# lijun9250lj/video-steganography-PCAMV

Measured on AMD Instinct MI355X. Metric: 1080p macroblocks/s (embed on), higher is better.
Workload: dtype u8

## Files before the change

### include/pcamv_gpu.h

```cpp
#ifndef PCAMV_GPU_H
#define PCAMV_GPU_H

#include <stddef.h>
#include <stdint.h>

#ifdef __cplusplus
extern "C" {
#endif

#define PCAMV_EINVAL  (-1)
#define PCAMV_ENODEV  (-2)
#define PCAMV_ENOMEM  (-3)
#define PCAMV_EHIP    (-4)
#define PCAMV_EUNSUP  (-5)

enum { PCAMV_ME_DIA = 0, PCAMV_ME_HEX = 1, PCAMV_ME_UMH = 2, PCAMV_ME_ESA = 3, PCAMV_ME_TESA = 4 };
enum { PCAMV_P_L0 = 4, PCAMV_P_8x8 = 5, PCAMV_P_SKIP = 6 };
enum { PCAMV_D_L0_4x4 = 0, PCAMV_D_L0_8x4 = 1, PCAMV_D_L0_4x8 = 2, PCAMV_D_L0_8x8 = 3,
       PCAMV_D_8x8 = 13, PCAMV_D_16x8 = 14, PCAMV_D_8x16 = 15, PCAMV_D_16x16 = 16 };
#define PCAMV_ANALYSE_I4x4      0x0001u
#define PCAMV_ANALYSE_PSUB16x16 0x0010u
#define PCAMV_ANALYSE_PSUB8x8   0x0020u

typedef struct pcamv_params_t {
    int32_t i_width, i_height;
    int32_t i_me_method;
    int32_t i_me_range;
    int32_t i_subpel_refine;
    int32_t i_mv_range;
    int32_t b_chroma_me;
    int32_t b_fast_pskip;
    int32_t b_dct_decimate;
    int32_t b_cabac;
    uint32_t inter;
    int32_t i_chroma_qp_offset;
    int32_t i_luma_deadzone[2];
    int32_t i_tscale;
    int32_t i_psy_rd;
} pcamv_params_t;

typedef struct pcamv_mb_t {
    int32_t i_type;
    int32_t i_partition;
    int32_t i_qp;
    uint8_t i_sub_partition[4];
    int8_t  ref[16];
    int16_t mv[16][2];
    int16_t mv_stego[16][2];
    int32_t inter_stego_cost[16];
    int16_t pskip_mv[2];
    int16_t mvr16[2];
    uint8_t used;
    uint8_t pad[3];
} pcamv_mb_t;

typedef struct pcamv_embed_t {
    int32_t  n;
    int32_t  m;
    int32_t  stc_ok;
    int32_t  num_flip;
    uint8_t *cover;
    float   *rho;
    uint8_t *message;
    uint8_t *stego;
    int8_t  *flip;
} pcamv_embed_t;

typedef struct pcamv_ctx pcamv_ctx_t;
typedef struct pcamv_batch pcamv_batch_t;

int  pcamv_gpu_open(const pcamv_params_t *param, int device, pcamv_ctx_t **ctx);
void pcamv_gpu_close(pcamv_ctx_t *ctx);
const char *pcamv_gpu_last_error(const pcamv_ctx_t *ctx);

int pcamv_gpu_upload_fenc(pcamv_ctx_t *ctx, const uint8_t *const plane[3], const int stride[3]);

int pcamv_gpu_set_ref(pcamv_ctx_t *ctx, const uint8_t *const plane[3], const int stride[3],
                      const int16_t *prev_mv, const int8_t *prev_ref);

int pcamv_gpu_get_ref_planes(pcamv_ctx_t *ctx, uint8_t *out, int *stride, int *lines);

int pcamv_gpu_analyse_pframe(pcamv_ctx_t *ctx, int qp, int embed, pcamv_mb_t *out_mb,
                             uint8_t *const recon[3]);

int pcamv_gpu_embed_pframe(pcamv_ctx_t *ctx, float emrate, const uint8_t *message, int message_len,
                           pcamv_embed_t *out);

int pcamv_gpu_final_mvs(pcamv_ctx_t *ctx, pcamv_mb_t *out_mb);

int pcamv_gpu_pass2_pframe(pcamv_ctx_t *ctx, const uint8_t *flips, int n_flips, pcamv_mb_t *out_final,
                           uint8_t *const recon[3], uint8_t *const deblocked[3]);

int pcamv_gpu_stc_extract(const uint8_t *stego, int n, int m, int matrixheight, uint8_t *message);
int pcamv_gpu_stc_extract_lcg(const uint8_t *stego, int n, int m, int matrixheight, int64_t *lcg, uint8_t *message);

int pcamv_gpu_parse_pslice_cabac(const uint8_t *slice_data, size_t len, int mb_w, int mb_h, int slice_qp, pcamv_mb_t *out_mb);
int pcamv_gpu_parse_pslice_cavlc(const uint8_t *slice_data, size_t len, int mb_w, int mb_h, pcamv_mb_t *out_mb);
int pcamv_gpu_nal_to_rbsp(const uint8_t *nal, size_t len, uint8_t *rbsp, size_t *rbsp_len, int *nal_ref_idc, int *nal_unit_type);
int pcamv_gpu_parse_pslice_cabac_at(const uint8_t *rbsp, size_t len, size_t start_bit, int mb_w, int mb_h, int slice_qp, pcamv_mb_t *out_mb);
int pcamv_gpu_parse_pslice_cavlc_at(const uint8_t *rbsp, size_t len, size_t start_bit, int mb_w, int mb_h, pcamv_mb_t *out_mb);

int pcamv_gpu_set_ref_device(pcamv_ctx_t *ctx, const void *y, const void *u, const void *v,
                             const void *prev_mv, const void *prev_ref);
#define PCAMV_PREV_FIELD_INTERNAL ((const void *)(uintptr_t)1)
int pcamv_gpu_set_fenc_device(pcamv_ctx_t *ctx, const void *y, const void *u, const void *v);
int pcamv_gpu_step_device(pcamv_ctx_t *ctx, int qp, float emrate, void *stream);
int pcamv_gpu_fetch_results(pcamv_ctx_t *ctx, pcamv_mb_t *out_mb, pcamv_embed_t *out);
int  pcamv_gpu_batch_create(pcamv_ctx_t *const *ctxs, int n, pcamv_batch_t **batch);
void pcamv_gpu_batch_destroy(pcamv_batch_t *batch);
int  pcamv_gpu_batch_step(pcamv_batch_t *batch, int qp, float emrate, void *stream);
int  pcamv_gpu_batch_kernel_time(pcamv_batch_t *batch, const char *kernel, double *avg_ms, int *launches, int reset);
const char *pcamv_gpu_batch_last_error(const pcamv_batch_t *batch);
int  pcamv_gpu_batch_set_closed_loop(pcamv_batch_t *batch, int on);
int  pcamv_gpu_recon_device(pcamv_ctx_t *ctx, void *planes[3]);
int  pcamv_gpu_fetch_recon(pcamv_ctx_t *ctx, uint8_t *const planes[3]);
const char *pcamv_gpu_batch_dominant_kernel(const pcamv_batch_t *batch);
int  pcamv_gpu_batch_copy_results_async(pcamv_batch_t *batch, void *dst_mb, size_t mb_stride, void *dst_flip, size_t flip_stride, void *stream);

int pcamv_gpu_kernel_time(pcamv_ctx_t *ctx, const char *kernel, double *avg_ms, int *launches, int reset);

int pcamv_gpu_block_costs(pcamv_ctx_t *ctx, int qp, int n, const int32_t *req, int32_t *out);

int pcamv_gpu_rd_probe(pcamv_ctx_t *ctx, int qp, int n, const uint8_t *req, int32_t *out);

int pcamv_gpu_embed_records(pcamv_ctx_t *ctx, const pcamv_mb_t *mbs, float emrate,
                            const uint8_t *message, int message_len, pcamv_embed_t *out);

int pcamv_gpu_trace_mb(pcamv_ctx_t *ctx, int mb);
int pcamv_gpu_trace_fetch(pcamv_ctx_t *ctx, int32_t *out);

int pcamv_gpu_debug_state_hash(pcamv_ctx_t *ctx, int enable);
int pcamv_gpu_debug_state_hash_fetch(pcamv_ctx_t *ctx, uint32_t *out);

int pcamv_gpu_abi_version(void);
#define PCAMV_FEATURE_PAYLOAD 0x1u
#define PCAMV_FEATURE_SLICE_PARSER 0x2u
#define PCAMV_FEATURE_SLICE_PARSER_CAVLC 0x4u
#define PCAMV_FEATURE_SLICE_WRITER 0x8u
#define PCAMV_FEATURE_SLICE_WRITER_CAVLC 0x10u
unsigned pcamv_gpu_features(void);

int pcamv_gpu_set_payload(pcamv_ctx_t *ctx, const uint8_t *bytes, int64_t n_bits);
int pcamv_gpu_set_payload_device(pcamv_ctx_t *ctx, const void *device_bytes, int64_t n_bits);
int pcamv_gpu_payload_tell(pcamv_ctx_t *ctx, int64_t *consumed_bits, int64_t *payload_bits);

int pcamv_gpu_rx_reserve(pcamv_ctx_t *ctx, int64_t n_bits);
int pcamv_gpu_rx_reset(pcamv_ctx_t *ctx);
int pcamv_gpu_rx_tell(pcamv_ctx_t *ctx, int64_t *received_bits, int64_t *reserved_bits);
int pcamv_gpu_rx_fetch(pcamv_ctx_t *ctx, uint8_t *bytes, int64_t n_bits);
int pcamv_gpu_batch_extract_step(pcamv_batch_t *batch, float emrate, void *stream);
int pcamv_gpu_extract_pframe(pcamv_ctx_t *ctx, const pcamv_mb_t *mbs, float emrate, uint8_t *bits_out, int32_t *n, int32_t *m);
int pcamv_gpu_batch_payload_check(pcamv_batch_t *batch, int64_t *diff);

int pcamv_gpu_parse_pslice_cabac_device(pcamv_ctx_t *ctx, const uint8_t *rbsp, size_t len, size_t start_bit, int slice_qp, pcamv_mb_t *out_mb);
typedef struct pcamv_slice_t { const uint8_t *rbsp; size_t len; size_t start_bit; int32_t slice_qp; } pcamv_slice_t;
int pcamv_gpu_batch_extract_slices(pcamv_batch_t *batch, const pcamv_slice_t *slices, float emrate, void *stream);
int pcamv_gpu_batch_extract_slices_device(pcamv_batch_t *batch, const void *bytes, size_t bytes_size, const int64_t *off, const int64_t *len,
                                          const int64_t *start_bit, const int32_t *slice_qp, float emrate, void *stream);
int pcamv_gpu_batch_slice_status(pcamv_batch_t *batch, int32_t *status);
int pcamv_gpu_debug_slice_records(pcamv_ctx_t *ctx, pcamv_mb_t *out_mb, int *guard_intact);

int pcamv_gpu_parse_pslice_cavlc_device(pcamv_ctx_t *ctx, const uint8_t *rbsp, size_t len, size_t start_bit, pcamv_mb_t *out_mb);
int pcamv_gpu_batch_extract_slices_cavlc(pcamv_batch_t *batch, const pcamv_slice_t *slices, float emrate, void *stream);
// ... 20 lines not shown
```

### video-steganography-pcamv_amd/csrc/pcamv_gpu.hip

```cpp
#include <hip/hip_runtime.h>
#include <math.h>
#include <stdarg.h>
#include <stdio.h>
#include <stdlib.h>
#include <string.h>
#include <new>
#include "pcamv_planes.hip.h"
#include "pcamv_kernels.hip.h"
#include "pcamv_embed.hip.h"
#include "pcamv_slice.hip.h"
#include "pcamv_host_tables.h"
#include "pcamv_mvsyntax.h"
#include "pcamv_rd_select.h"

#define PCAMV_ABI_VERSION 3
#define NEV 32
#define NRING 8
#define NKEV 16
enum { KT_ANALYSE, KT_EMBED_PREPARE, KT_EXTRACT_PREPARE, KT_EXTRACT_BITS, KT_PAYLOAD_CHECK, KT_PARSE_PSLICE, KT_PARSE_PSLICE_CAVLC, KT_WRITE_PSLICE, KT_WRITE_PSLICE_CAVLC, KT_N };
#define PCAMV_FEATURES (PCAMV_FEATURE_PAYLOAD | PCAMV_FEATURE_SLICE_PARSER | PCAMV_FEATURE_SLICE_PARSER_CAVLC | PCAMV_FEATURE_SLICE_WRITER | \
                        PCAMV_FEATURE_SLICE_WRITER_CAVLC)
#define SLICE_GUARD_MBS 4
#define NSTAGE 2
enum { ST_PLANES = 1, ST_ANALYSE = 2, ST_EMBED = 4, ST_PASS2 = 8 };
// ... 518 lines not shown
    *k_out = k;
    return 0;
}
static int stage_release(pcamv_batch *b, StageRing &R, int k, hipStream_t st)
{
    HIPCHK(b, hipEventRecord(R.done[k], st));
    R.used[k] = 1;
    return 0;
}
static int stage_send(pcamv_batch *b, StageRing &R, int k, size_t total, hipStream_t st)
{
    HIPCHK(b, hipMemcpyAsync(R.d[k], R.h[k], total, hipMemcpyHostToDevice, st));
    return stage_release(b, R, k, st);
}
static int batch_push_descs(pcamv_batch *b, hipStream_t st, const FrameDev **dF, const EmbedDev **dE, int *slot_out)
{
    int slot;
    TRY(ring_take(b, b->ring, &slot));
    FrameDev *hF = b->h_F + (size_t)slot * b->n; EmbedDev *hE = b->h_E + (size_t)slot * b->n;
    for (int i = 0; i < b->n; i++) { hF[i] = b->ctx[i]->F; hF[i].self = b->d_F + (size_t)slot * b->n + i; hE[i] = b->ctx[i]->E; }
    HIPCHK(b, hipMemcpyAsync(b->d_F + (size_t)slot * b->n, hF, sizeof(FrameDev) * b->n, hipMemcpyHostToDevice, st));
    HIPCHK(b, hipMemcpyAsync(b->d_E + (size_t)slot * b->n, hE, sizeof(EmbedDev) * b->n, hipMemcpyHostToDevice, st));
    *dF = b->d_F + (size_t)slot * b->n; *dE = b->d_E + (size_t)slot * b->n; *slot_out = slot;
    return 0;
}

template <class Launch> static void diag_launch(int n_diag, const FrameDev &F, Launch launch)
{
    for (int d = 0; d < n_diag; d++) {
        int y_lo = d - (F.mb_w - 1); y_lo = y_lo > 0 ? (y_lo + 1) >> 1 : 0;
        int y_hi = d / 2; if (y_hi > F.mb_h - 1) y_hi = F.mb_h - 1;
        int cnt = y_hi - y_lo + 1;
        if (cnt <= 0) continue;
        launch(cnt, d);
    }
}

static int kt_begin(pcamv_batch *b, int k, hipStream_t st)
{
    KTimer &T = b->kt[k];
    if (T.made < 0) return -1;
    if (!T.made) {
        for (int i = 0; i < T.cap; i++) if (hipEventCreate(&T.e0[i]) != hipSuccess || hipEventCreate(&T.e1[i]) != hipSuccess) { T.made = -1; return -1; }
        T.made = 1;
    }
    hipEventRecord(T.e0[T.head], st);
    return T.head;
}
static void kt_end(pcamv_batch *b, int k, int ev, hipStream_t st)
{
    KTimer &T = b->kt[k];
    if (ev < 0) return;
    hipEventRecord(T.e1[ev], st);
    T.head = (T.head + 1) % T.cap; if (T.n < T.cap) T.n++;
}

static void pass2_takes_rec(pcamv_ctx *c)
{
    c->F.rec_is_pass1 = c->rec_pristine;
    c->rec_pristine = 0;
}

static int batch_launch(pcamv_batch *b, int what, hipStream_t st)
{
    HIPCHK(b, hipSetDevice(b->device));
    TRY(batch_live(b));
    for (int i = 0; i < b->n; i++) {
        pcamv_ctx *c = b->ctx[i];
        if ((what & ST_ANALYSE) && c->prev_internal) {
            const int wr = !c->last_field;
            c->F.mv = wr ? c->d_mv_b : c->d_mv; c->F.ref8 = wr ? c->d_ref8_b : c->d_ref8;
            c->F.prev_mv = wr ? c->d_mv : c->d_mv_b; c->F.prev_ref = wr ? c->d_ref8 : c->d_ref8_b;
        }
        if (what & ST_ANALYSE) c->last_field = c->F.mv == c->d_mv_b;
        if (what & ST_ANALYSE) c->rec_pristine = 1;
        if (what & ST_PASS2) pass2_takes_rec(c);
        else c->F.rec_is_pass1 = 0;
    }
    const FrameDev *dF; const EmbedDev *dE; int slot;
    TRY(batch_push_descs(b, st, &dF, &dE, &slot));
    const FrameDev &F = b->ctx[0]->F;
    const unsigned G = (unsigned)b->n;
    if (what & ST_PLANES) {
        dim3 g((F.stride / 4 + HP_THREADS - 1) / HP_THREADS, (F.lines + HP_ROWS - 1) / HP_ROWS, G);
        hipLaunchKernelGGL(k_hpel, g, dim3(HP_THREADS), 0, st, dF);
        dim3 gc((F.cstride / 4 + 255) / 256, F.clines, 2 * G);
        hipLaunchKernelGGL(k_chroma_pad, gc, dim3(256), 0, st, dF);
    }
    if (what & ST_ANALYSE) {
        for (int i = 0; i < b->n; i++) b->ctx[i]->last = b;
        if (b->sched_flow) {
            hipLaunchKernelGGL(k_flow_init, dim3((b->fl.total + 255) / 256), dim3(256), 0, st, b->fl);
            const int ev = kt_begin(b, KT_ANALYSE, st);
            if (b->b_mbrd) b->rd->launch((unsigned)b->flow_waves, st, dF, b->fl);
            else if (b->b_tesa) pcamv_launch_flow_tesa((unsigned)b->flow_waves, st, dF, b->fl);
            else hipLaunchKernelGGL(k_analyse_flow, dim3(b->flow_waves), dim3(64), 0, st, dF, b->fl);
            kt_end(b, KT_ANALYSE, ev, st);
        } else {
            const int ev = kt_begin(b, KT_ANALYSE, st);
            diag_launch(b->n_diag, F, [&](int cnt, int d) { hipLaunchKernelGGL(k_search_diag<0>, dim3(cnt, G), dim3(64), 0, st, dF, d); });
            kt_end(b, KT_ANALYSE, ev, st);
            hipLaunchKernelGGL(k_rca, dim3(F.n_mb * b->slots_per_mb, G), dim3(64), 0, st, dF, b->slots_per_mb);
            hipLaunchKernelGGL(k_encode, dim3(F.n_mb, G), dim3(64), 0, st, dF);
        }
    }
    if (what & ST_EMBED) {
        const int ev = kt_begin(b, KT_EMBED_PREPARE, st);
        hipLaunchKernelGGL(k_embed_prepare, dim3(G), dim3(1024), 0, st, dE);
        kt_end(b, KT_EMBED_PREPARE, ev, st);
        if (b->stc_ns == 4) hipLaunchKernelGGL(k_stc_forward<4>, dim3(G), dim3(256), 0, st, dE);
        else hipLaunchKernelGGL(k_stc_forward<2>, dim3(G), dim3(512), 0, st, dE);
        hipLaunchKernelGGL(k_stc_backward, dim3(G), dim3(64), 0, st, dE);
        hipLaunchKernelGGL(k_mb_flips, dim3((F.n_mb + 255) / 256, G), dim3(256), 0, st, dE);
    }
    if (what & ST_PASS2) {
        if (b->sched_flow) {
            hipLaunchKernelGGL(k_flow_init, dim3((b->fl2.total + 255) / 256), dim3(256), 0, st, b->fl2);
            hipLaunchKernelGGL(k_pass2_deblock_flow, dim3(b->flow2_waves), dim3(64), 0, st, dF, b->fl2);
        } else {
            diag_launch(b->n_diag, F, [&](int cnt, int d) { pcamv_launch_pass2_diag(P2D_PASS2 | P2D_DEBLOCK, cnt, G, st, dF, d); });
        }
    }
    TRY(launched(b));
    return ring_release(b, b->ring, slot, st);
}
static int flow_check(pcamv_batch *b)
{
    if (!b || !b->sched_flow) return 0;
    unsigned bad = 0;
    HIPCHK(b, hipMemcpy(&bad, b->fl.ctr + FLOW_ERR, sizeof(bad), hipMemcpyDeviceToHost));
    if (bad) {
        hipMemset(b->fl.ctr + FLOW_ERR, 0, sizeof(unsigned));
        return fail(b, PCAMV_EHIP, "dataflow kernel: queue wait timed out (results of the last step are incomplete)");
    }
    return 0;
}
static int ctx_launch(pcamv_ctx *c, int what) { return on_behalf(c, c->self, batch_launch(c->self, what, c->stream)); }

extern "C" int pcamv_gpu_set_ref(pcamv_ctx_t *c, const uint8_t *const plane[3], const int stride[3], const int16_t *prev_mv, const int8_t *prev_ref)
{
    if (!c || !plane || !stride) return PCAMV_EINVAL;
    HIPCHK(c, hipSetDevice(c->device));
    for (int i = 0; i < 3; i++) {
        int w = c->F.w >> !!i, h = c->F.h >> !!i;
        HIPCHK(c, hipMemcpy2D(c->d_raw[i], w, plane[i], stride[i], w, h, hipMemcpyHostToDevice));
        c->F.raw[i] = c->d_raw[i];
    }
    c->F.have_prev = prev_mv != NULL && prev_ref != NULL && c->p.i_tscale != 0;
    c->F.ref_is_inter = prev_mv != NULL && prev_ref != NULL;
    c->prev_internal = 0;
    c->F.mv = c->d_mv; c->F.ref8 = c->d_ref8;
    c->F.prev_mv = c->d_prev_mv; c->F.prev_ref = c->d_prev_ref;
    if (c->F.have_prev) {
        HIPCHK(c, hipMemcpy(c->d_prev_mv, prev_mv, (size_t)c->F.n_mb * 64, hipMemcpyHostToDevice));
        HIPCHK(c, hipMemcpy(c->d_prev_ref, prev_ref, (size_t)c->F.n_mb * 4, hipMemcpyHostToDevice));
    }
    TRY(ctx_launch(c, ST_PLANES));
    HIPCHK(c, hipStreamSynchronize(c->stream));
    return 0;
}
extern "C" int pcamv_gpu_set_ref_device(pcamv_ctx_t *c, const void *y, const void *u, const void *v, const void *prev_mv, const void *prev_ref)
{
    if (!c || !y || !u || !v) return PCAMV_EINVAL;
    c->F.have_prev = prev_mv != NULL && prev_ref != NULL && c->p.i_tscale != 0;
    c->F.ref_is_inter = prev_mv != NULL && prev_ref != NULL;
    c->prev_internal = prev_mv == PCAMV_PREV_FIELD_INTERNAL;
    if (c->F.have_prev && !c->prev_internal) { c->F.prev_mv = (const int16_t *)prev_mv; c->F.prev_ref = (const int8_t *)prev_ref; c->F.mv = c->d_mv; c->F.ref8 = c->d_ref8; }
    c->F.raw[0] = (const uint8_t *)y; c->F.raw[1] = (const uint8_t *)u; c->F.raw[2] = (const uint8_t *)v;
    return 0;
}

extern "C" int pcamv_gpu_get_ref_planes(pcamv_ctx_t *c, uint8_t *out, int *stride, int *lines)
{
    if (!c || !out) return PCAMV_EINVAL;
    HIPCHK(c, hipSetDevice(c->device));
    HIPCHK(c, hipDeviceSynchronize());
    const size_t psz = (size_t)c->F.plane_size;
    HostTmp<uint8_t> tmp(4 * psz);
    if (!tmp) return fail(c, PCAMV_EHIP, "out of host memory");
    HIPCHK(c, hipMemcpy(tmp, c->F.luma_base, 4 * psz, hipMemcpyDeviceToHost));
    for (int k = 0; k < 4; k++)
        for (int y = 0; y < c->F.lines; y++)
            for (int x = 0; x < c->F.stride; x++)
                out[((size_t)k * c->F.lines + y) * c->F.stride + x] = tmp[k * psz + (size_t)y * PCAMV_LROW + x + (size_t)(x / PCAMV_LSW) * c->F.lskip];
    if (stride) *stride = c->F.stride;
    if (lines) *lines = c->F.lines;
    return 0;
}

extern "C" int pcamv_gpu_analyse_pframe(pcamv_ctx_t *c, int qp, int embed, pcamv_mb_t *out_mb, uint8_t *const recon[3])
{
    if (!c || !out_mb) return PCAMV_EINVAL;
    HIPCHK(c, hipSetDevice(c->device));
    TRY(ensure_qp(c, qp));
    c->F.embed = embed;
    TRY(ctx_launch(c, ST_ANALYSE));
    HIPCHK(c, hipStreamSynchronize(c->stream));
    TRY(on_behalf(c, c->self, flow_check(c->self)));
    HIPCHK(c, hipMemcpy(out_mb, c->F.rec_mb, (size_t)c->F.n_mb * sizeof(pcamv_mb_t), hipMemcpyDeviceToHost));
    if (recon)
        for (int i = 0; i < 3; i++)
            if (recon[i]) HIPCHK(c, hipMemcpy(recon[i], c->F.rec[i], ((size_t)c->F.w * c->F.h) >> (i ? 2 : 0), hipMemcpyDeviceToHost));
    return 0;
}

static int fetch_embed(pcamv_ctx *c, pcamv_embed_t *out)
{
    int hdr[8];
    HIPCHK(c, hipDeviceSynchronize());
    HIPCHK(c, hipMemcpy(hdr, c->E.hdr, sizeof(hdr), hipMemcpyDeviceToHost));
    out->n = hdr[0]; out->m = hdr[1]; out->stc_ok = hdr[2]; out->num_flip = hdr[3];
    if (out->n < 0 || out->m < 0 || out->n > c->cap) return fail(c, PCAMV_EHIP, "embed header corrupt");
    const int m_copy = out->m < c->cap ? out->m : c->cap;
    if (out->cover && out->n) HIPCHK(c, hipMemcpy(out->cover, c->E.cover, out->n, hipMemcpyDeviceToHost));
    if (out->rho && out->n) HIPCHK(c, hipMemcpy(out->rho, c->E.rho, (size_t)out->n * 4, hipMemcpyDeviceToHost));
    if (out->stego && out->n) HIPCHK(c, hipMemcpy(out->stego, c->E.stego, out->n, hipMemcpyDeviceToHost));
    if (out->flip && out->n) HIPCHK(c, hipMemcpy(out->flip, c->d_flip, out->n, hipMemcpyDeviceToHost));
    if (out->message && m_copy) HIPCHK(c, hipMemcpy(out->message, c->E.message, m_copy, hipMemcpyDeviceToHost));
    return 0;
}

static int embed_stage(pcamv_ctx *c, float emrate, const uint8_t *message, int message_len, pcamv_embed_t *out)
{
    if (message) {
        if (message_len < 0 || message_len > c->cap) return fail(c, PCAMV_EINVAL, "message_len");
        HIPCHK(c, hipMemcpy(c->d_user_msg, message, message_len, hipMemcpyHostToDevice));
        c->E.user_message = c->d_user_msg; c->E.user_message_len = message_len;
    } else { c->E.user_message = NULL; c->E.user_message_len = 0; }
    c->E.emrate = emrate;
    TRY(ctx_launch(c, ST_EMBED));
    return fetch_embed(c, out);
}
extern "C" int pcamv_gpu_embed_pframe(pcamv_ctx_t *c, float emrate, const uint8_t *message, int message_len, pcamv_embed_t *out)
{
    if (!c || !out || emrate <= 0) return PCAMV_EINVAL;
    HIPCHK(c, hipSetDevice(c->device));
    return embed_stage(c, emrate, message, message_len, out);
}
extern "C" int pcamv_gpu_embed_records(pcamv_ctx_t *c, const pcamv_mb_t *mbs, float emrate, const uint8_t *message, int message_len, pcamv_embed_t *out)
{
    if (!c || !mbs || !out || emrate <= 0) return PCAMV_EINVAL;
    HIPCHK(c, hipSetDevice(c->device));
    HIPCHK(c, hipDeviceSynchronize());
    HIPCHK(c, hipMemcpy(c->F.rec_mb, mbs, (size_t)c->F.n_mb * sizeof(pcamv_mb_t), hipMemcpyHostToDevice));
    return embed_stage(c, emrate, message, message_len, out);
}

static int mb_carrier_slots(const pcamv_mb_t *mb, int slots[16])
{
    int n = 0;
    if (!mb->used) return 0;
    if (mb->i_type == PCAMV_P_8x8) {
        for (int i = 0; i < 4; i++)
            switch (mb->i_sub_partition[i]) {
            case PCAMV_D_L0_8x8: slots[n++] = i * 4; break;
            case PCAMV_D_L0_4x8: slots[n++] = i * 4; slots[n++] = i * 4 + 1; break;
            case PCAMV_D_L0_8x4: slots[n++] = i * 4; slots[n++] = i * 4 + 2; break;
            default: for (int j = 0; j < 4; j++) slots[n++] = i * 4 + j; break;
            }
    } else if (mb->i_type == PCAMV_P_L0) {
        slots[n++] = 0;
        if (mb->i_partition == PCAMV_D_8x16) slots[n++] = 4;
        else if (mb->i_partition == PCAMV_D_16x8) slots[n++] = 8;
    }
    return n;
}

extern "C" int pcamv_gpu_pass2_pframe(pcamv_ctx_t *c, const uint8_t *flips, int n_flips, pcamv_mb_t *out_final,
                                      uint8_t *const recon[3], uint8_t *const deblocked[3])
// ... 782 lines not shown
```

### video-steganography-pcamv_amd/csrc/pcamv_planes.hip.h

```cpp
#ifndef PCAMV_PLANES_HIP_H
#define PCAMV_PLANES_HIP_H
#include "pcamv_common.h"
#include "pcamv_prims_gpu.h"

static __global__ void __launch_bounds__(256) k_chroma_pad(const FrameDev *__restrict__ Fs)
{
    const FrameDev &F = Fs[blockIdx.z >> 1];
    const int pl = blockIdx.z & 1;
    const uint8_t *__restrict__ src = F.raw[1 + pl];
    uint8_t *__restrict__ dst = F.chroma_base[pl];
    const int w = F.w >> 1, h = F.h >> 1, cstride = F.cstride, clines = F.clines;
    const int x = 4 * (blockIdx.x * blockDim.x + threadIdx.x), y = blockIdx.y;
    if (x >= cstride || y >= clines) return;
    const uint8_t *rowp = src + (size_t)clip3i(y - PCAMV_CPAD, 0, h - 1) * w;
    const int gx = x - PCAMV_CPAD;
    uint32_t v;
    if (gx < 0 || gx >= w) v = rowp[gx < 0 ? 0 : w - 1] * 0x01010101u;
    else if (((uintptr_t)src & 3) == 0) v = *(const uint32_t *)(rowp + gx);
    else v = rowp[gx] | rowp[gx + 1] << 8 | rowp[gx + 2] << 16 | (uint32_t)rowp[gx + 3] << 24;
    *(uint32_t *)(dst + (size_t)y * cstride + x) = v;
}

#define HP_ROWS 16
#define HP_THREADS 128
__device__ __forceinline__ void hpel_load_row(const uint8_t *__restrict__ rowp, int eg0, int W, bool fast, uint32_t d[3])
{
    if (fast) {
        const uint32_t *q = (const uint32_t *)(rowp + eg0 - 4);
        d[0] = q[0]; d[1] = q[1]; d[2] = q[2];
    } else {
#pragma unroll
        for (int i = 0; i < 3; i++) {
            uint32_t v = 0;
#pragma unroll
            for (int b = 0; b < 4; b++) v |= (uint32_t)rowp[clip3i(eg0 - 4 + 4 * i + b, 0, W - 1)] << (8 * b);
            d[i] = v;
        }
    }
}
static __global__ void __launch_bounds__(HP_THREADS) k_hpel(const FrameDev *__restrict__ Fs)
{
    const FrameDev &F = Fs[blockIdx.z];
    const uint8_t *__restrict__ src = F.raw[0];
    uint8_t *__restrict__ planes = F.luma_base;
    const int W = F.w, H = F.h, stride = F.stride, lines = F.lines;
    const int x0 = 4 * (blockIdx.x * HP_THREADS + threadIdx.x), yb = blockIdx.y * HP_ROWS;
    if (x0 >= stride) return;
    const int gx = x0 - PCAMV_PAD, eg0 = clip3i(gx, -4, W);
    const int rep = gx < -4 ? 0 : gx > W ? 3 : -1;
    const bool fast = eg0 >= 4 && eg0 + 8 <= W && ((uintptr_t)src & 3) == 0;
    const size_t psz = (size_t)F.plane_size;
    const unsigned strip = PCAMV_LSTRIP_OF(x0);
    const size_t strip_o = (size_t)x0 + (size_t)strip * (size_t)F.lskip;
    const bool dup = strip > 0 && (unsigned)x0 == strip * PCAMV_LSW;
    uint32_t w[6][3];
    uint32_t of = 0, oh = 0, ov = 0, oc = 0;
    int ey_prev = 0;
    for (int y = yb; y < yb + HP_ROWS && y < lines; y++) {
        const int ey = clip3i(y - PCAMV_PAD, -8, H + 7);
        if (y == yb || ey != ey_prev) {
            if (y == yb) {
#pragma unroll
                for (int k = 0; k < 5; k++) hpel_load_row(src + (size_t)clip3i(ey - 2 + k, 0, H - 1) * W, eg0, W, fast, w[k]);
            } else {
#pragma unroll
                for (int k = 0; k < 5; k++) { w[k][0] = w[k + 1][0]; w[k][1] = w[k + 1][1]; w[k][2] = w[k + 1][2]; }
            }
            hpel_load_row(src + (size_t)clip3i(ey + 3, 0, H - 1) * W, eg0, W, fast, w[5]);
            ey_prev = ey;
            int v[9], b2[9];
#pragma unroll
            for (int j = 0; j < 9; j++) {
                const int q = (j + 2) >> 2, sh = 8 * ((j + 2) & 3);
#define HPB(k) ((int)(w[k][q] >> sh & 255))
                v[j] = HPB(0) + HPB(5) - 5 * (HPB(1) + HPB(4)) + 20 * (HPB(2) + HPB(3));
                b2[j] = HPB(2);
#undef HPB
            }
            of = w[2][1]; oh = ov = oc = 0;
#pragma unroll
            for (int k = 0; k < 4; k++) {
                const int th = b2[k] + b2[k + 5] - 5 * (b2[k + 1] + b2[k + 4]) + 20 * (b2[k + 2] + b2[k + 3]);
                const int tc = v[k] + v[k + 5] - 5 * (v[k + 1] + v[k + 4]) + 20 * (v[k + 2] + v[k + 3]);
                oh |= clamp_u8((th + 16) >> 5) << (8 * k);
                ov |= clamp_u8((v[k + 2] + 16) >> 5) << (8 * k);
                oc |= clamp_u8((tc + 512) >> 10) << (8 * k);
            }
            if (rep >= 0) {
                const int sh = 8 * rep;
                of = (of >> sh & 255) * 0x01010101u; oh = (oh >> sh & 255) * 0x01010101u;
                ov = (ov >> sh & 255) * 0x01010101u; oc = (oc >> sh & 255) * 0x01010101u;
            }
        }
        const size_t o = (size_t)y * PCAMV_LROW + strip_o;
        *(uint32_t *)(planes + o) = of;
        if (F.luma_raster) *(uint32_t *)(F.luma_raster + (size_t)y * stride + x0) = of;
        *(uint32_t *)(planes + psz + o) = oh;
        *(uint32_t *)(planes + 2 * psz + o) = ov;
        *(uint32_t *)(planes + 3 * psz + o) = oc;
        if (dup) {
            const size_t o2 = o - (size_t)F.lskip;
            *(uint32_t *)(planes + o2) = of;
            *(uint32_t *)(planes + psz + o2) = oh;
            *(uint32_t *)(planes + 2 * psz + o2) = ov;
            *(uint32_t *)(planes + 3 * psz + o2) = oc;
        }
    }
}
#endif
```

### video-steganography-pcamv_amd/pcamv_amd/api.py

```python
import ctypes as C
import os
import subprocess

import numpy as np

_PKG = os.path.dirname(os.path.dirname(os.path.abspath(__file__)))
_CSRC = os.path.join(_PKG, "csrc")

ME_NAMES = {"dia": 0, "hex": 1, "umh": 2, "esa": 3, "tesa": 4}
P_L0, P_8x8, P_SKIP = 4, 5, 6
I4x4, PSUB16x16, PSUB8x8 = 0x01, 0x10, 0x20


class PcamvError(RuntimeError):
    pass


class Params(C.Structure):
    _fields_ = [("i_width", C.c_int32), ("i_height", C.c_int32), ("i_me_method", C.c_int32),
                ("i_me_range", C.c_int32), ("i_subpel_refine", C.c_int32), ("i_mv_range", C.c_int32),
                ("b_chroma_me", C.c_int32), ("b_fast_pskip", C.c_int32), ("b_dct_decimate", C.c_int32),
                ("b_cabac", C.c_int32), ("inter", C.c_uint32), ("i_chroma_qp_offset", C.c_int32),
                ("i_luma_deadzone", C.c_int32 * 2), ("i_tscale", C.c_int32), ("i_psy_rd", C.c_int32)]

# ... 235 lines not shown
FEATURE_SLICE_PARSER = 0x2
FEATURE_SLICE_PARSER_CAVLC = 0x4
FEATURE_SLICE_WRITER = 0x8
FEATURE_SLICE_WRITER_CAVLC = 0x10


def features():
    lib = load_library()
    lib.pcamv_gpu_features.restype = C.c_uint
    return lib.pcamv_gpu_features()


def pack_bits(bits):
    bits = np.ascontiguousarray(bits, np.uint8) & 1
    return np.packbits(bits, bitorder="big"), len(bits)


def unpack_bits(packed, n_bits):
    packed = np.ascontiguousarray(packed, np.uint8)
    if n_bits > 8 * len(packed):
        raise PcamvError(f"{n_bits} bits asked of {len(packed)} bytes")
    return np.unpackbits(packed, bitorder="big")[:n_bits]


def _is_device_tensor(x):
    return hasattr(x, "data_ptr") and hasattr(x, "is_cuda")


class Encoder:

    def __init__(self, params, device=0):
        self.lib = load_library()
        self.p = params
        self.w, self.h = params.i_width, params.i_height
        self.n_mb = (self.w // 16) * (self.h // 16)
        ctx = C.c_void_p()
        rc = self.lib.pcamv_gpu_open(C.byref(params), device, C.byref(ctx))
        if rc:
            names = {-1: "invalid parameter", -2: "no HIP device (there is no CPU fallback)", -3: "out of memory",
                     -4: "HIP error", -5: "unsupported (subme >= 8, tesa with me_range > 16, ... are not on the GPU path)"}
            raise PcamvError(f"pcamv_gpu_open failed: {names.get(rc, rc)}")
        self.ctx = ctx

    def _chk(self, rc, what):
        if rc:
            raise PcamvError(f"{what} failed ({rc}): {self.lib.pcamv_gpu_last_error(self.ctx).decode()}")

    def close(self):
        if getattr(self, "ctx", None):
            self.lib.pcamv_gpu_close(self.ctx)
            self.ctx = None

    def __del__(self):
        try:
            self.close()
        except Exception:
            pass

    def _planes(self, y, u, v):
        arrs = [np.ascontiguousarray(a, np.uint8) for a in (y, u, v)]
        ptrs = (C.c_void_p * 3)(*[a.ctypes.data for a in arrs])
        strides = (C.c_int * 3)(*[a.shape[1] for a in arrs])
        return arrs, ptrs, strides

    def upload_fenc(self, y, u, v):
        keep, ptrs, strides = self._planes(y, u, v)
        self._chk(self.lib.pcamv_gpu_upload_fenc(self.ctx, ptrs, strides), "upload_fenc")

    def set_ref(self, y, u, v, prev_mv=None, prev_ref=None):
        keep, ptrs, strides = self._planes(y, u, v)
        if prev_mv is not None:
            prev_mv = np.ascontiguousarray(prev_mv, np.int16)
            prev_ref = np.ascontiguousarray(prev_ref, np.int8)
        self._chk(self.lib.pcamv_gpu_set_ref(self.ctx, ptrs, strides, _p(prev_mv), _p(prev_ref)), "set_ref")

    def ref_planes(self):
        stride = (self.w + 64 + 15) & ~15
        out = np.zeros((4, self.h + 64, stride), np.uint8)
        st, ln = C.c_int(), C.c_int()
        self._chk(self.lib.pcamv_gpu_get_ref_planes(self.ctx, _p(out), C.byref(st), C.byref(ln)), "get_ref_planes")
        assert st.value == stride and ln.value == self.h + 64
        return out

    def analyse_pframe(self, qp, embed=1, want_recon=True):
        mbs = np.zeros(self.n_mb, MB_DTYPE)
        rec = [np.zeros((self.h, self.w), np.uint8), np.zeros((self.h // 2, self.w // 2), np.uint8),
               np.zeros((self.h // 2, self.w // 2), np.uint8)]
        ptrs = (C.c_void_p * 3)(*[a.ctypes.data for a in rec]) if want_recon else None
        self._chk(self.lib.pcamv_gpu_analyse_pframe(self.ctx, qp, embed, _p(mbs), ptrs), "analyse_pframe")
        return mbs, rec

    def _embed_bufs(self):
        cap = 16 * self.n_mb
        arr = dict(cover=np.zeros(cap, np.uint8), rho=np.zeros(cap, np.float32), message=np.zeros(cap, np.uint8),
                   stego=np.zeros(cap, np.uint8), flip=np.zeros(cap, np.int8))
        e = _Embed(0, 0, 0, 0, *[arr[k].ctypes.data for k in ("cover", "rho", "message", "stego", "flip")])
        return arr, e

    @staticmethod
    def _embed_out(arr, e):
        out = {k: v[:e.n].copy() for k, v in arr.items()}
        out["message"] = arr["message"][:e.m].copy()
        out.update(n=e.n, m=e.m, stc_ok=e.stc_ok, num_flip=e.num_flip)
        return out

    def embed_pframe(self, emrate, message=None):
        arr, e = self._embed_bufs()
        if message is not None:
            message = np.ascontiguousarray(message, np.uint8)
        self._chk(self.lib.pcamv_gpu_embed_pframe(self.ctx, C.c_float(emrate), _p(message),
                                                  0 if message is None else len(message), C.byref(e)), "embed_pframe")
        return self._embed_out(arr, e)

    def embed_records(self, mbs, emrate, message=None):
        mbs = np.ascontiguousarray(mbs, MB_DTYPE)
        if len(mbs) != self.n_mb:
            raise PcamvError(f"{len(mbs)} records for a picture of {self.n_mb} macroblocks")
        arr, e = self._embed_bufs()
        if message is not None:
            message = np.ascontiguousarray(message, np.uint8)
        self.lib.pcamv_gpu_embed_records.argtypes = [C.c_void_p, C.c_void_p, C.c_float, C.c_void_p, C.c_int, C.c_void_p]
        self._chk(self.lib.pcamv_gpu_embed_records(self.ctx, _p(mbs), emrate, _p(message), 0 if message is None else len(message), C.byref(e)),
                  "embed_records")
        return self._embed_out(arr, e)

    def set_payload(self, payload, n_bits=None):
        self.lib.pcamv_gpu_set_payload.argtypes = [C.c_void_p, C.c_void_p, C.c_int64]
        self.lib.pcamv_gpu_set_payload_device.argtypes = [C.c_void_p, C.c_void_p, C.c_int64]
        self._payload_keep = None
        if payload is None:
            return self._chk(self.lib.pcamv_gpu_set_payload(self.ctx, None, 0), "set_payload")
        if _is_device_tensor(payload):
            if not payload.is_cuda or payload.element_size() != 1 or not payload.is_contiguous():
                raise PcamvError("a borrowed payload is a contiguous uint8 tensor on the device")
            n_bits = 8 * payload.numel() if n_bits is None else n_bits
            if n_bits > 8 * payload.numel():
                raise PcamvError("n_bits beyond the tensor")
            self._payload_keep = payload
            return self._chk(self.lib.pcamv_gpu_set_payload_device(self.ctx, C.c_void_p(payload.data_ptr()), n_bits), "set_payload_device")
        data = np.frombuffer(payload, np.uint8) if isinstance(payload, (bytes, bytearray)) else np.ascontiguousarray(payload, np.uint8)
        n_bits = 8 * len(data) if n_bits is None else n_bits
        if n_bits > 8 * len(data):
            raise PcamvError("n_bits beyond the buffer")
        self._chk(self.lib.pcamv_gpu_set_payload(self.ctx, _p(data), n_bits), "set_payload")

    def payload_tell(self):
        used, total = C.c_int64(), C.c_int64()
        self._chk(self.lib.pcamv_gpu_payload_tell(self.ctx, C.byref(used), C.byref(total)), "payload_tell")
        return used.value, total.value

    def rx_reserve(self, n_bits):
        self.lib.pcamv_gpu_rx_reserve.argtypes = [C.c_void_p, C.c_int64]
        self._chk(self.lib.pcamv_gpu_rx_reserve(self.ctx, n_bits), "rx_reserve")

    def rx_reset(self):
        self._chk(self.lib.pcamv_gpu_rx_reset(self.ctx), "rx_reset")

    def rx_tell(self):
        got, cap = C.c_int64(), C.c_int64()
        self._chk(self.lib.pcamv_gpu_rx_tell(self.ctx, C.byref(got), C.byref(cap)), "rx_tell")
        return got.value, cap.value

    def received(self, n_bits=None, packed=False):
        self.lib.pcamv_gpu_rx_fetch.argtypes = [C.c_void_p, C.c_void_p, C.c_int64]
        if n_bits is None:
            got, cap = self.rx_tell()
# ... 281 lines not shown
```

Baseline: 25.79 million.

## Stage hpel output in LDS for 128-bit strip writes and widen chroma pad

The half-pel plane kernel is remapped so each 64-thread block handles eight luma strips, eight lanes per strip. Four rows of full/h/v/c results are staged in shared memory and written out as 128-bit stores instead of scattered 32-bit ones, and the duplicate strip-boundary writes are dropped. The chroma pad kernel now writes 16 bytes per thread across four rows per block. A new API exports the raw strip layout for testing, which adds code but no hot-path work. The rewritten indexing risks layout mismatches, and the planes stage is a small part of the frame pipeline.

```diff
diff --git a/include/pcamv_gpu.h b/include/pcamv_gpu.h
--- a/include/pcamv_gpu.h
+++ b/include/pcamv_gpu.h
@@ -79,6 +79,8 @@
                       const int16_t *prev_mv, const int8_t *prev_ref);
 
 int pcamv_gpu_get_ref_planes(pcamv_ctx_t *ctx, uint8_t *out, int *stride, int *lines);
+
+int pcamv_gpu_get_ref_strips(pcamv_ctx_t *ctx, uint8_t *out, size_t cap, size_t *luma_bytes, size_t *chroma_bytes);
 
 int pcamv_gpu_analyse_pframe(pcamv_ctx_t *ctx, int qp, int embed, pcamv_mb_t *out_mb,
                              uint8_t *const recon[3]);
diff --git a/video-steganography-pcamv_amd/csrc/pcamv_gpu.hip b/video-steganography-pcamv_amd/csrc/pcamv_gpu.hip
--- a/video-steganography-pcamv_amd/csrc/pcamv_gpu.hip
+++ b/video-steganography-pcamv_amd/csrc/pcamv_gpu.hip
@@ -624,10 +624,10 @@
     const FrameDev &F = b->ctx[0]->F;
     const unsigned G = (unsigned)b->n;
     if (what & ST_PLANES) {
-        dim3 g((F.stride / 4 + HP_THREADS - 1) / HP_THREADS, (F.lines + HP_ROWS - 1) / HP_ROWS, G);
+        dim3 g(((F.stride + PCAMV_LSW - 1) / PCAMV_LSW + 7) / 8, (F.lines + HP_ROWS - 1) / HP_ROWS, G);
         hipLaunchKernelGGL(k_hpel, g, dim3(HP_THREADS), 0, st, dF);
-        dim3 gc((F.cstride / 4 + 255) / 256, F.clines, 2 * G);
-        hipLaunchKernelGGL(k_chroma_pad, gc, dim3(256), 0, st, dF);
+        dim3 gc((F.cstride / 16 * CP_ROWS + CP_THREADS - 1) / CP_THREADS, (F.clines + CP_ROWS - 1) / CP_ROWS, 2 * G);
+        hipLaunchKernelGGL(k_chroma_pad, gc, dim3(CP_THREADS), 0, st, dF);
     }
     if (what & ST_ANALYSE) {
         for (int i = 0; i < b->n; i++) b->ctx[i]->last = b;
@@ -727,6 +727,21 @@
                 out[((size_t)k * c->F.lines + y) * c->F.stride + x] = tmp[k * psz + (size_t)y * PCAMV_LROW + x + (size_t)(x / PCAMV_LSW) * c->F.lskip];
     if (stride) *stride = c->F.stride;
     if (lines) *lines = c->F.lines;
+    return 0;
+}
+
+extern "C" int pcamv_gpu_get_ref_strips(pcamv_ctx_t *c, uint8_t *out, size_t cap, size_t *luma_bytes, size_t *chroma_bytes)
+{
+    if (!c) return PCAMV_EINVAL;
+    HIPCHK(c, hipSetDevice(c->device));
+    HIPCHK(c, hipDeviceSynchronize());
+    const size_t lb = 4 * (size_t)c->F.plane_size, csz = (size_t)c->F.cstride * c->F.clines;
+    if (luma_bytes) *luma_bytes = lb;
+    if (chroma_bytes) *chroma_bytes = 2 * csz;
+    if (!out) return 0;
+    if (cap < lb + 2 * csz) return fail(c, PCAMV_EINVAL, "get_ref_strips: %zu bytes offered, %zu needed", cap, lb + 2 * csz);
+    HIPCHK(c, hipMemcpy(out, c->F.luma_base, lb, hipMemcpyDeviceToHost));
+    for (int k = 0; k < 2; k++) HIPCHK(c, hipMemcpy(out + lb + k * csz, c->F.chroma_base[k], csz, hipMemcpyDeviceToHost));
     return 0;
 }
 
diff --git a/video-steganography-pcamv_amd/csrc/pcamv_planes.hip.h b/video-steganography-pcamv_amd/csrc/pcamv_planes.hip.h
--- a/video-steganography-pcamv_amd/csrc/pcamv_planes.hip.h
+++ b/video-steganography-pcamv_amd/csrc/pcamv_planes.hip.h
@@ -3,30 +3,43 @@
 #include "pcamv_common.h"
 #include "pcamv_prims_gpu.h"
 
-static __global__ void __launch_bounds__(256) k_chroma_pad(const FrameDev *__restrict__ Fs)
+typedef uint32_t u32x4 __attribute__((ext_vector_type(4)));
+typedef __attribute__((address_space(1))) u32x4 *gp128w;
+typedef __attribute__((address_space(1))) uint32_t *gp32w;
+typedef const __attribute__((address_space(1))) uint32_t *gp32;
+#define CP_ROWS 4
+#define CP_THREADS 256
+static __global__ void __launch_bounds__(CP_THREADS) k_chroma_pad(const FrameDev *__restrict__ Fs)
 {
     const FrameDev &F = Fs[blockIdx.z >> 1];
     const int pl = blockIdx.z & 1;
     const uint8_t *__restrict__ src = F.raw[1 + pl];
     uint8_t *__restrict__ dst = F.chroma_base[pl];
     const int w = F.w >> 1, h = F.h >> 1, cstride = F.cstride, clines = F.clines;
-    const int x = 4 * (blockIdx.x * blockDim.x + threadIdx.x), y = blockIdx.y;
-    if (x >= cstride || y >= clines) return;
+    const int per_row = cstride >> 4;
+    const int i = blockIdx.x * CP_THREADS + threadIdx.x;
+    const int y = blockIdx.y * CP_ROWS + i / per_row, x = 16 * (i % per_row);
+    if (i >= per_row * CP_ROWS || y >= clines) return;
     const uint8_t *rowp = src + (size_t)clip3i(y - PCAMV_CPAD, 0, h - 1) * w;
-    const int gx = x - PCAMV_CPAD;
-    uint32_t v;
-    if (gx < 0 || gx >= w) v = rowp[gx < 0 ? 0 : w - 1] * 0x01010101u;
-    else if (((uintptr_t)src & 3) == 0) v = *(const uint32_t *)(rowp + gx);
-    else v = rowp[gx] | rowp[gx + 1] << 8 | rowp[gx + 2] << 16 | (uint32_t)rowp[gx + 3] << 24;
-    *(uint32_t *)(dst + (size_t)y * cstride + x) = v;
+    const bool aligned = ((uintptr_t)src & 3) == 0;
+    uint32_t v[4];
+#pragma unroll
+    for (int k = 0; k < 4; k++) {
+        const int gx = x + 4 * k - PCAMV_CPAD;
+        if (gx < 0 || gx >= w) v[k] = rowp[gx < 0 ? 0 : w - 1] * 0x01010101u;
+        else if (aligned) v[k] = *(const uint32_t *)(rowp + gx);
+        else v[k] = rowp[gx] | rowp[gx + 1] << 8 | rowp[gx + 2] << 16 | (uint32_t)rowp[gx + 3] << 24;
+    }
+    *(gp128w)(dst + (size_t)y * cstride + x) = u32x4{v[0], v[1], v[2], v[3]};
 }
 
 #define HP_ROWS 16
-#define HP_THREADS 128
+#define HP_THREADS 64
+#define HP_TILE 40
 __device__ __forceinline__ void hpel_load_row(const uint8_t *__restrict__ rowp, int eg0, int W, bool fast, uint32_t d[3])
 {
     if (fast) {
-        const uint32_t *q = (const uint32_t *)(rowp + eg0 - 4);
+        const gp32 q = (gp32)(rowp + eg0 - 4);
         d[0] = q[0]; d[1] = q[1]; d[2] = q[2];
     } else {
 #pragma unroll
@@ -40,19 +53,21 @@
 }
 static __global__ void __launch_bounds__(HP_THREADS) k_hpel(const FrameDev *__restrict__ Fs)
 {
+    __shared__ uint32_t tile[4][8][HP_TILE];
     const FrameDev &F = Fs[blockIdx.z];
     const uint8_t *__restrict__ src = F.raw[0];
     uint8_t *__restrict__ planes = F.luma_base;
     const int W = F.w, H = F.h, stride = F.stride, lines = F.lines;
-    const int x0 = 4 * (blockIdx.x * HP_THREADS + threadIdx.x), yb = blockIdx.y * HP_ROWS;
-    if (x0 >= stride) return;
+    const int t = threadIdx.x >> 3, d = threadIdx.x & 7;
+    const int strip = blockIdx.x * 8 + t, yb = blockIdx.y * HP_ROWS;
+    if (strip * PCAMV_LSW >= stride) return;
+    const int x0 = strip * PCAMV_LSW + 4 * d;
     const int gx = x0 - PCAMV_PAD, eg0 = clip3i(gx, -4, W);
     const int rep = gx < -4 ? 0 : gx > W ? 3 : -1;
     const bool fast = eg0 >= 4 && eg0 + 8 <= W && ((uintptr_t)src & 3) == 0;
     const size_t psz = (size_t)F.plane_size;
-    const unsigned strip = PCAMV_LSTRIP_OF(x0);
-    const size_t strip_o = (size_t)x0 + (size_t)strip * (size_t)F.lskip;
-    const bool dup = strip > 0 && (unsigned)x0 == strip * PCAMV_LSW;
+    uint8_t *const line0 = planes + (size_t)strip * PCAMV_LROW * (size_t)lines + 16 * d;
+    const bool raster = F.luma_raster && d < 7 && x0 < stride;
     uint32_t w[6][3];
     uint32_t of = 0, oh = 0, ov = 0, oc = 0;
     int ey_prev = 0;
@@ -92,18 +107,18 @@
                 ov = (ov >> sh & 255) * 0x01010101u; oc = (oc >> sh & 255) * 0x01010101u;
             }
         }
-        const size_t o = (size_t)y * PCAMV_LROW + strip_o;
-        *(uint32_t *)(planes + o) = of;
-        if (F.luma_raster) *(uint32_t *)(F.luma_raster + (size_t)y * stride + x0) = of;
-        *(uint32_t *)(planes + psz + o) = oh;
-        *(uint32_t *)(planes + 2 * psz + o) = ov;
-        *(uint32_t *)(planes + 3 * psz + o) = oc;
-        if (dup) {
-            const size_t o2 = o - (size_t)F.lskip;
-            *(uint32_t *)(planes + o2) = of;
-            *(uint32_t *)(planes + psz + o2) = oh;
-            *(uint32_t *)(planes + 2 * psz + o2) = ov;
-            *(uint32_t *)(planes + 3 * psz + o2) = oc;
+        if (raster) *(gp32w)(F.luma_raster + (size_t)y * stride + x0) = of;
+        const int r = y & 3;
+        tile[0][t][8 * r + d] = of; tile[1][t][8 * r + d] = oh; tile[2][t][8 * r + d] = ov; tile[3][t][8 * r + d] = oc;
+        if (r == 3) {
+            PCAMV_WAVE_SYNC();
+            u32x4 ln[4];
+#pragma unroll
+            for (int k = 0; k < 4; k++) ln[k] = *(const u32x4 *)&tile[k][t][4 * d];
+            PCAMV_WAVE_SYNC();
+            uint8_t *const o = line0 + (size_t)(y - 3) * PCAMV_LROW;
+#pragma unroll
+            for (int k = 0; k < 4; k++) *(gp128w)(o + k * psz) = ln[k];
         }
     }
 }
diff --git a/video-steganography-pcamv_amd/pcamv_amd/api.py b/video-steganography-pcamv_amd/pcamv_amd/api.py
--- a/video-steganography-pcamv_amd/pcamv_amd/api.py
+++ b/video-steganography-pcamv_amd/pcamv_amd/api.py
@@ -341,6 +341,16 @@
         assert st.value == stride and ln.value == self.h + 64
         return out
 
+    def ref_strips(self):
+        fn = self.lib.pcamv_gpu_get_ref_strips
+        fn.argtypes = [C.c_void_p, C.c_void_p, C.c_size_t, C.POINTER(C.c_size_t), C.POINTER(C.c_size_t)]
+        lb, cb = C.c_size_t(), C.c_size_t()
+        self._chk(fn(self.ctx, None, 0, C.byref(lb), C.byref(cb)), "get_ref_strips")
+        out = np.zeros(lb.value + cb.value, np.uint8)
+        self._chk(fn(self.ctx, _p(out), out.size, C.byref(lb), C.byref(cb)), "get_ref_strips")
+        lines, clines = self.h + 64, self.h // 2 + 32
+        return out[:lb.value].reshape(4, -1, lines, 32), out[lb.value:].reshape(2, clines, -1)
+
     def analyse_pframe(self, qp, embed=1, want_recon=True):
         mbs = np.zeros(self.n_mb, MB_DTYPE)
         rec = [np.zeros((self.h, self.w), np.uint8), np.zeros((self.h // 2, self.w // 2), np.uint8),
```

After: 26.08 million (median of 6 runs). 1.01x the previous value.
